# gabrieldemarmiesse/mojo-simdjson

Hardware: AMD Instinct MI355X
Metric: stage-1 GB/s JSON ingested (+ % HBM3E peak), 1/2/4/8 MI355X (higher is better)
Workload: dtype u8

## Files before the change

### mojo_simdjson_amd/csrc/lane_math.h

```cpp
#pragma once
#include <stdint.h>

#if defined(__HIPCC__)
#define MSJ_HD __host__ __device__ __forceinline__
#else
#define MSJ_HD static inline
#endif

namespace msj {

MSJ_HD uint32_t perm(uint32_t s0, uint32_t s1, uint32_t sel) {
#if defined(__HIP_DEVICE_COMPILE__)
    return __builtin_amdgcn_perm(s0, s1, sel);
#else
    uint64_t d = ((uint64_t)s0 << 32) | s1;
    uint32_t r = 0;
    for (int i = 0; i < 4; i++) {
        uint32_t s = (sel >> (8 * i)) & 0xFF;
        r |= (uint32_t)((d >> (8 * (s & 7))) & 0xFF) << (8 * i);
    }
    return r;
#endif
}

// ... 195 lines not shown
#else
    return (uint32_t)__builtin_clzll(inv);
#endif
}

MSJ_HD uint64_t escape_tt0(uint64_t backslash) {
    const uint64_t ODD = 0xAAAAAAAAAAAAAAAAull;
    const uint32_t lo = (uint32_t)backslash, hi = (uint32_t)(backslash >> 32);
    uint32_t sl;
#if defined(__HIP_DEVICE_COMPILE__)
    asm("v_add_u32_e32 %0, %1, %1" : "=v"(sl) : "v"(lo));
    const uint32_t sh = __builtin_amdgcn_alignbit(hi, lo, 31);
#else
    sl = lo << 1;
    const uint32_t sh = (hi << 1) | (lo >> 31);
#endif
    return (u64(sl, sh) | ODD) - backslash;
}
MSJ_HD uint32_t escape_out0(uint64_t tt, uint64_t backslash) {
    return lut3<MSJ_TT((TA ^ TB) & TC)>((uint32_t)(tt >> 32), 0xAAAAAAAAu, (uint32_t)(backslash >> 32)) >> 31;
}
MSJ_HD uint64_t unescaped_quotes0(uint64_t quote_chr, uint64_t tt) {
    return lut3<MSJ_TT(TA & ~(TB ^ TC))>(quote_chr, tt, 0xAAAAAAAAAAAAAAAAull);
}

struct Utf8Leads {
    uint64_t lead234, lead34, lead4;
    uint64_t l3, hi2, f;
};

MSJ_HD Utf8Leads utf8_leads(const uint64_t p[8]) {
    const uint64_t b3 = p[3], b4 = p[4], b5 = p[5], b6 = p[6], b7 = p[7];
    Utf8Leads u;
    u.hi2 = b7 & b6;
    u.f = lut3<MSJ_TT(TA & TB & TC)>(u.hi2, b5, b4);
    u.l3 = lut3<MSJ_TT(TA & TB & ~TC)>(u.hi2, b5, b4);
    u.lead4 = lut3<MSJ_TT(TA & ~TB)>(u.f, b3, b3);
    u.lead234 = lut3<MSJ_TT(TA & ~(TB & TC))>(u.hi2, u.f, b3);
    u.lead34 = u.l3 | u.lead4;
    return u;
}

MSJ_HD uint32_t utf8_special_top(const uint64_t p[8], const Utf8Leads &u) {
    const uint32_t t = 63;
    const uint32_t b0 = (uint32_t)(p[0] >> t) & 1u, b1 = (uint32_t)(p[1] >> t) & 1u, b2 = (uint32_t)(p[2] >> t) & 1u;
    const uint32_t b3 = (uint32_t)(p[3] >> t) & 1u, l3 = (uint32_t)(u.l3 >> t) & 1u, l4 = (uint32_t)(u.lead4 >> t) & 1u;
    const uint32_t z210 = !(b2 | b1 | b0), n101 = b2 & !b1 & b0, n100 = b2 & !b1 & !b0;
    return ((l3 & !b3 & z210) << 6) | ((l3 & b3 & n101) << 7) | ((l4 & z210) << 8) | ((l4 & n100) << 9);
}

MSJ_HD uint32_t utf8_carry_out(const uint64_t p[8], const Utf8Leads &u) {
    return (uint32_t)(u.lead234 >> 63) | ((uint32_t)(u.lead34 >> 62) << 1) | ((uint32_t)(u.lead4 >> 61) << 3) |
           utf8_special_top(p, u);
}

MSJ_HD uint32_t utf8_boundary_error(uint32_t carry_in, uint32_t first_b5, uint32_t first_b4) {
    const uint32_t n5 = first_b5 & 1u, n54 = (first_b5 | first_b4) & 1u;
    return (((carry_in >> 6) & 1u) & (n5 ^ 1u)) |
           (((carry_in >> 7) & 1u) & n5) |
           (((carry_in >> 8) & 1u) & (n54 ^ 1u)) |
           (((carry_in >> 9) & 1u) & n54);
}

template <int K>
MSJ_HD uint64_t shl_in(uint64_t x, uint32_t low) {
    const uint32_t lo = (uint32_t)x, hi = (uint32_t)(x >> 32);
#if defined(__HIP_DEVICE_COMPILE__)
    const uint32_t nh = __builtin_amdgcn_alignbit(hi, lo, 32 - K);
#else
    const uint32_t nh = (hi << K) | (lo >> (32 - K));
#endif
    return u64((lo << K) | low, nh);
}

struct Utf8Shifted {
    uint64_t exp1, exp2, exp3;
    uint64_t nb5, nb54;
};

MSJ_HD uint64_t utf8_errors_shifted(const uint64_t p[8], const Utf8Leads &u, const Utf8Shifted &s, uint64_t *pair_bad) {
    const uint64_t b0 = p[0], b1 = p[1], b2 = p[2], b3 = p[3];
    const uint64_t b4 = p[4], b5 = p[5], b6 = p[6], b7 = p[7];
    const uint64_t cont = lut3<MSJ_TT(TA & ~TB)>(b7, b6, b6);
    const uint64_t e12 = s.exp1 | s.exp2;
    uint64_t err = lut3<MSJ_TT((TA | TB) ^ TC)>(e12, s.exp3, cont);
    const uint64_t x567 = lut3<MSJ_TT(TA & (TB | TC))>(b2, b1, b0);
    const uint64_t f5ff = lut3<MSJ_TT(TA & (TB | TC))>(u.f, b3, x567);
    const uint64_t z432 = lut3<MSJ_TT(~TA & ~TB & ~TC)>(b4, b3, b2);
    const uint64_t w = lut3<MSJ_TT(TA & ~TB & ~TC)>(z432, b1, b5);
    const uint64_t c0c1 = u.hi2 & w;
    err = lut3<MSJ_TT(TA | TB | TC)>(err, f5ff, c0c1);
    const uint64_t z210 = lut3<MSJ_TT(~TA & ~TB & ~TC)>(b2, b1, b0);
    const uint64_t m10 = lut3<MSJ_TT(TA & ~TB)>(b2, b1, b1);
    const uint64_t t1 = lut3<MSJ_TT(TA & ~TB & ~TC)>(u.l3, b3, s.nb5);
    const uint64_t t2 = lut3<MSJ_TT((TA & ~TB) | TC)>(u.lead4, s.nb54, t1);
    const uint64_t u1 = lut3<MSJ_TT(TA & TB & TC)>(u.l3, b3, s.nb5);
    const uint64_t v1 = u.lead4 & s.nb54;
    const uint64_t sel = lut3<MSJ_TT((TC & TA) | (~TC & TB))>(u1, v1, b0);
    const uint64_t lo_bad = z210 & t2;
    *pair_bad = lut3<MSJ_TT(TA | (TB & TC))>(lo_bad, m10, sel);
    return err;
}

MSJ_HD uint64_t utf8_errors(const uint64_t p[8], const Utf8Leads &u, uint32_t carry_in, uint32_t next_b5,
                            uint32_t next_b4, bool have_next) {
    const uint32_t c = carry_in;
// ... 53 lines not shown
```

### mojo_simdjson_amd/csrc/stage1_kernel.hip

```cpp
#include <hip/hip_runtime.h>
#include <stddef.h>
#include <stdint.h>

#include "../../include/msj_stage1.h"
#include "lane_math.h"
#include "stage1_kernel.h"

namespace msj {

constexpr uint32_t kPrioCoord = 2;
constexpr uint32_t kPrioEmit = 3;
constexpr uint32_t kPrioCompute = 0;
constexpr uint32_t kPrioCompute2 = 1;

constexpr uint64_t kAgg = 1ull << 62;
constexpr uint64_t kPre = 2ull << 62;

__device__ __forceinline__ uint64_t ld_desc(const uint64_t *p) {
    return __hip_atomic_load(p, __ATOMIC_RELAXED, __HIP_MEMORY_SCOPE_AGENT);
}
__device__ __forceinline__ void st_desc(uint64_t *p, uint64_t v) {
    __hip_atomic_store(p, v, __ATOMIC_RELAXED, __HIP_MEMORY_SCOPE_AGENT);
}

// ... 92 lines not shown
__device__ __forceinline__ uint32_t cin_internal_error(const KernelArgs &a) {
    return (a.flags & kFlagCarryByValue) ? 0u : a.carry_in->internal_error & 1u;
}
__device__ __forceinline__ msj_carry cin_all(const KernelArgs &a) {
    if (!(a.flags & kFlagCarryByValue)) return *a.carry_in;
    msj_carry c;
    c.count = c.bytes = 0;
    c.in_string = a.carry_bits & 1u;
    c.next_is_escaped = (a.carry_bits >> 1) & 1u;
    c.prev_scalar = (a.carry_bits >> 2) & 1u;
    c.unescaped_error = c.utf8_error = c.internal_error = c.capacity_error = 0;
    c.code = 0;
    for (int k = 0; k < 4; k++) c.reserved[k] = 0;
    return c;
}

struct WaitClock {
    uint32_t spins = 0, t0 = 0;
    __device__ __forceinline__ bool expired(const uint32_t wait_ticks) {
        if ((++spins & 15u) != 0u) return false;
        const uint32_t now = (uint32_t)__builtin_amdgcn_s_memrealtime();
        if (spins == 16u) {
            t0 = now;
            return false;
        }
        return now - t0 > wait_ticks;
    }
    __device__ __forceinline__ void restart() { spins = 0; }
};

__device__ __forceinline__ uint64_t wait_desc(const uint64_t *p, const uint32_t wait_ticks, uint32_t *timeout) {
    uint64_t d = uniform64(ld_desc(p));
    WaitClock clk;
    while ((d >> 62) == 0ull) {
        __builtin_amdgcn_s_sleep(2);
        d = uniform64(ld_desc(p));
        if (clk.expired(wait_ticks)) {
            *timeout = 1;
            break;
        }
    }
    return d;
}

__device__ __forceinline__ void lds_wave_sync_early() {
    asm volatile("s_waitcnt lgkmcnt(0)" ::: "memory");
    __builtin_amdgcn_fence(__ATOMIC_RELEASE, "wavefront");
    __builtin_amdgcn_wave_barrier();
    __builtin_amdgcn_fence(__ATOMIC_ACQUIRE, "wavefront");
}

struct Block {
    uint4 q[4];
    uint32_t wb;
};

template <bool kCoalesced, bool kNt = false>
__device__ __forceinline__ void load_block(const KernelArgs &a, const uint32_t tile, const uint32_t (&lane_off)[4],
                                           const uint32_t lane, Block &b) {
    const uint32_t len32 = (uint32_t)a.len;
    const uint32_t tile_off = tile * kTileBytes;
    const uint8_t *base = a.buf + tile_off;
    const uint32_t lim = ((len32 - 1u) & ~15u) - tile_off;
#pragma unroll
    for (int k = 0; k < 4; k++) {
        const uint32_t off = lane_off[k] < lim ? lane_off[k] : lim;
        if (kCoalesced) {
            typedef uint32_t u32x4 __attribute__((ext_vector_type(4)));
            const u32x4 *src = reinterpret_cast<const u32x4 *>(base + off);
            const u32x4 v = kNt ? __builtin_nontemporal_load(src) : *src;
            b.q[k] = make_uint4(v.x, v.y, v.z, v.w);
        } else {
            b.q[k] = *reinterpret_cast<const uint4 *>(base + off);
        }
    }
    const bool have_window = (tile > 0) || (a.flags & kFlagHasPrefix);
    const uint8_t *wbase = have_window ? base - 64 : a.buf;
    const uint32_t wlim = have_window ? 63u : len32 - 1u;
    b.wb = wbase[lane < wlim ? lane : wlim];
}

struct ChunkAddr {
    uint32_t wr, rd, sw16;
};
__device__ __forceinline__ ChunkAddr chunk_addresses(const uint32_t *stage, const uint32_t lane) {
    const uint32_t s0 = (uint32_t)(uintptr_t)stage;
    ChunkAddr c;
    c.wr = s0 + 64u * (lane >> 2) + 16u * ((lane & 3u) ^ ((lane >> 3) & 3u));
    c.rd = s0 + 64u * lane;
    c.sw16 = 16u * ((lane >> 1) & 3u);
    return c;
}
__device__ __forceinline__ void chunks_to_block(Block &b, const ChunkAddr &ca) {
    typedef uint32_t u32x4 __attribute__((ext_vector_type(4)));
    typedef __attribute__((address_space(3))) u32x4 *lds_u32x4_ptr;
#pragma unroll
    for (int k = 0; k < 4; k++) {
        const u32x4 v = {b.q[k].x, b.q[k].y, b.q[k].z, b.q[k].w};
        *(lds_u32x4_ptr)(uintptr_t)(ca.wr + 1024u * k) = v;
    }
    lds_wave_sync_early();
#pragma unroll
    for (int c = 0; c < 4; c++) {
        const u32x4 v = *(lds_u32x4_ptr)(uintptr_t)(ca.rd + (ca.sw16 ^ (16u * c)));
        b.q[c] = make_uint4(v.x, v.y, v.z, v.w);
    }
}

template <bool kNt>
__device__ __forceinline__ void load_range(const KernelArgs &a, const uint32_t lo, const uint32_t wave,
                                           const uint32_t (&lane_off)[4], const uint32_t lane, Block (&blk)[kBatch]) {
    const uint32_t ntiles = a.ntiles;
#pragma unroll
    for (uint32_t j = 0; j < kBatch; j++) {
        const uint32_t t = lo + kWaves * j + wave;
        load_block<true, kNt>(a, t < ntiles ? t : ntiles - 1u, lane_off, lane, blk[j]);
    }
}
constexpr uint32_t kNtMaxIndices = 3000;
constexpr uint32_t kNtMinTiles = 98304;

__device__ __forceinline__ void touch_block(Block &b) {
#pragma unroll
    for (int k = 0; k < 4; k++)
        asm volatile("" : "+v"(b.q[k].x), "+v"(b.q[k].y), "+v"(b.q[k].z), "+v"(b.q[k].w));
    asm volatile("" : "+v"(b.wb));
}
__device__ __forceinline__ void touch_u64(uint64_t &v) {
    uint32_t lo = (uint32_t)v, hi = (uint32_t)(v >> 32);
    asm volatile("" : "+v"(lo), "+v"(hi));
    v = ((uint64_t)hi << 32) | lo;
}

__device__ __forceinline__ uint32_t ticket_request(unsigned int *ctr, uint32_t lane, uint32_t count) {
    uint32_t ret = 0;
    if (lane == 0)
        asm volatile("global_atomic_add %0, %1, %2, off sc0" : "=v"(ret) : "v"(ctr), "v"(count) : "memory");
    return ret;
}
__device__ __forceinline__ uint32_t ticket_value(uint32_t reg) {
    asm volatile("s_waitcnt vmcnt(0)" ::: "memory");
    return bcast(reg, 0);
}
__device__ __forceinline__ uint32_t ticket_range(uint32_t k, uint32_t shard, uint32_t shards) {
    return (k - (shard == 0u ? 1u : 0u)) * shards + shard;
}

__device__ __forceinline__ void scatter_bits32(uint32_t t, uint32_t lds_byte_addr, uint32_t nbits, uint32_t value_base) {
    uint32_t lo, hi, tm1;
    uint64_t save;
    const uint32_t back = lds_byte_addr + 4u * nbits - 128u;
    const uint32_t vb31 = value_base + 31u;
    const uint32_t topbit = 0x80000000u;
    asm volatile(
        "s_mov_b64 %[save], exec\n"
        ".set msj_sb_k, 0\n"
        ".rept 16\n"
        "v_cmpx_ne_u32_e32 vcc, 0, %[t]\n"
        "s_cbranch_execz 1f\n"
        "v_ffbl_b32_e32 %[lo], %[t]\n"
        "v_ffbh_u32_e32 %[hi], %[t]\n"
        "v_add_u32_e32 %[tm1], -1, %[t]\n"
        "v_or_b32_e32 %[lo], %[lo], %[vb]\n"
        "ds_write_b32 %[front], %[lo] offset:4*msj_sb_k\n"
        "v_sub_u32_e32 %[lo], %[vb31], %[hi]\n"
        "v_lshrrev_b32_e32 %[hi], %[hi], %[top]\n"
        "ds_write_b32 %[back], %[lo] offset:124-4*msj_sb_k\n"
        "v_bitop3_b32 %[t], %[t], %[tm1], %[hi] bitop3:0x40\n"
        ".set msj_sb_k, msj_sb_k+1\n"
        ".endr\n"
        "1:\n"
        "s_mov_b64 exec, %[save]\n"
        : [t] "+v"(t), [lo] "=&v"(lo), [hi] "=&v"(hi), [tm1] "=&v"(tm1), [save] "=&s"(save)
        : [front] "v"(lds_byte_addr), [back] "v"(back), [vb] "v"(value_base), [vb31] "v"(vb31), [top] "v"(topbit)
        : "vcc", "memory");
}

static_assert(offsetof(Shared, stage) >= 128, "scatter_bits32 addresses the back slots from 128 bytes below the lane's end slot");

struct Pending {
    uint64_t T0, T1;
    uint32_t excl;
    uint32_t tile_cnt;
};

struct TileCarry {
    uint32_t e_in, ps_in, u8_in;
    bool resolved;
};
__device__ __forceinline__ TileCarry window_carries(const KernelArgs &a, const uint32_t tile, const uint32_t wb,
                                                    const uint32_t carry0) {
    TileCarry c;
    const bool have_window = (tile > 0) || (a.flags & kFlagHasPrefix);
    const uint32_t b1 = bcast(wb, 63), b2 = bcast(wb, 62), b3 = bcast(wb, 61);
    c.u8_in = 0;
    if (have_window && ((b1 | b2 | b3) & 0x80u)) {
        const uint32_t l1 = (b1 >= 0xC0u && b1 < 0xF8u), l1_34 = (b1 >= 0xE0u && b1 < 0xF8u);
        const uint32_t l1_4 = (b1 >= 0xF0u && b1 < 0xF8u);
        const uint32_t l2_34 = (b2 >= 0xE0u && b2 < 0xF8u), l2_4 = (b2 >= 0xF0u && b2 < 0xF8u);
        const uint32_t l3_4 = (b3 >= 0xF0u && b3 < 0xF8u);
        c.u8_in = l1 | (l2_34 << 1) | (l1_34 << 2) | (l3_4 << 3) | (l2_4 << 4) | (l1_4 << 5) |
                  ((uint32_t)(b1 == 0xE0u) << 6) | ((uint32_t)(b1 == 0xEDu) << 7) |
                  ((uint32_t)(b1 == 0xF0u) << 8) | ((uint32_t)(b1 == 0xF4u) << 9);
    }
    const uint64_t WB = __ballot(wb == 0x5Cu);
    constexpr uint64_t ODD = 0xAAAAAAAAAAAAAAAAull;
    const uint64_t t = (((WB << 1) | ODD) - WB) ^ ODD;
    const uint32_t esc1 = (uint32_t)((t ^ WB) >> 63);
    constexpr uint64_t kNsLo = (1ull << 0x09) | (1ull << 0x0A) | (1ull << 0x0C) | (1ull << 0x0D) |
                               (1ull << 0x1A) | (1ull << 0x20) | (1ull << 0x2C) | (1ull << 0x3A);
    constexpr uint64_t kNsHi = (1ull << (0x5B - 64)) | (1ull << (0x5D - 64)) |
                               (1ull << (0x7B - 64)) | (1ull << (0x7D - 64));
    const uint64_t tab = (b1 & 0x40u) ? kNsHi : kNsLo;
    const uint32_t nonscalar = (uint32_t)(tab >> (b1 & 63u)) & (uint32_t)(b1 < 0x80u);
    c.e_in = (uint32_t)((t & WB) >> 63);
    c.ps_in = ~nonscalar & 1u & ((b1 == 0x22u) ? esc1 : 1u);
    c.resolved = (WB | (1ull << 63)) != ~0ull;
    if (tile == 0) {
        c.e_in = carry0 & 1u;
        c.ps_in = (carry0 >> 1) & 1u;
        c.resolved = true;
    }
    return c;
}

__device__ __forceinline__ Pending compute_tile(const KernelArgs &a, const uint32_t tile,
                                                const uint32_t lane, const Block &blk, const uint32_t carry0,
                                                uint32_t &timeout, uint64_t &agg_word, const uint32_t exact = 0u) {
    const uint32_t len = (uint32_t)a.len;
    MSJ_STAMP(tile, 1);
    uint32_t x[16];
#pragma unroll
    for (int k = 0; k < 4; k++) {
        x[4 * k + 0] = blk.q[k].x;
        x[4 * k + 1] = blk.q[k].y;
        x[4 * k + 2] = blk.q[k].z;
        x[4 * k + 3] = blk.q[k].w;
    }
    TileCarry tc = window_carries(a, tile, blk.wb, carry0);
    if (exact & 1u) {
        tc.e_in = (exact >> 1) & 1u;
        tc.ps_in = (exact >> 2) & 1u;
        tc.resolved = true;
    }
    const uint32_t skip = tile == 0 ? (a.flags >> kFlagSkipShift) & 15u : 0u;
    const bool partial = tile * kTileBytes + kTileBytes > len;

    MSJ_STAMP(tile, 2);
    uint64_t p[8];
    bitplanes(x, p);
    Classes cls;
    uint64_t valid = ~0ull;
    if (!partial && !skip) {
        cls = classify(p, ~0ull);
    } else {
        const uint32_t blk_off = tile * kTileBytes + lane * 64u;
        if (blk_off >= len)
            valid = 0ull;
        else if (len - blk_off < 64u)
            valid = (1ull << (len - blk_off)) - 1ull;
        if (lane == 0) valid &= ~0ull << skip;
#pragma unroll
        for (int k = 0; k < 8; k++) p[k] &= valid;
        cls = classify(p, valid);
    }
    const uint64_t nonascii = __ballot(((uint32_t)p[7] | (uint32_t)(p[7] >> 32)) != 0u);

    const uint64_t qb = cls.quote_chr | cls.backslash;
    const bool quiet = __ballot(((uint32_t)qb | (uint32_t)(qb >> 32)) != 0u) == 0ull && !partial && tc.resolved;
    uint64_t quote = 0, in_string0 = 0, escaped = 0;
    uint32_t tile_e_out = 0, tile_par = 0;
    if (!quiet) {
        const uint64_t tt = escape_tt0(cls.backslash);
        const uint64_t G = __ballot(escape_out0(tt, cls.backslash) != 0u);
        const uint64_t Pm = __ballot(((uint32_t)cls.backslash & (uint32_t)(cls.backslash >> 32)) == 0xFFFFFFFFu);
        quote = unescaped_quotes0(cls.quote_chr, tt);
        const uint64_t add_a = G | Pm, add_b = G;
        uint64_t add_s = add_a + add_b + tc.e_in;
        uint64_t carries = add_s ^ add_a ^ add_b;
        MSJ_STAMP(tile, 3);
        if (carries != 0ull || partial || !tc.resolved) {
            if (!tc.resolved) {
                uint32_t to = 0;
                const uint64_t d = wait_desc(&a.ws[kDescOffset + tile - 1], a.wait_ticks, &to);
                if (to) timeout = 1;
                tc.e_in = (uint32_t)(d >> 58) & 1u;
                tc.ps_in = (uint32_t)(d >> 57) & 1u;
                add_s = add_a + add_b + tc.e_in;
                carries = add_s ^ add_a ^ add_b;
            }
            const uint64_t B0 = __ballot(((uint32_t)cls.backslash & 1u) != 0u);
            if ((carries & B0) == 0ull && !partial) {
                const bool starts_escaped = __builtin_amdgcn_inverse_ballot_w64(carries);
                const uint32_t qlo = (uint32_t)quote;
                quote = u64(starts_escaped ? qlo & ~1u : qlo, (uint32_t)(quote >> 32));
            } else {
                uint32_t lane_e_out;
                escaped = escaped_mask(cls.backslash, (uint32_t)(carries >> lane) & 1u, &lane_e_out);
                quote = cls.quote_chr & ~escaped;
            }
        }
        const uint64_t S0 = prefix_xor(quote);
        tile_e_out = (uint32_t)(((add_a & add_b) | ((add_a | add_b) & ~add_s)) >> 63);
        const uint64_t PM = __ballot((int32_t)(uint32_t)(S0 >> 32) < 0);
        const uint32_t lane_par = lanes_below(PM);
        tile_par = (uint32_t)__popcll(PM) & 1u;
        const uint32_t lane_in32 = (uint32_t)__builtin_amdgcn_sbfe((int)lane_par, 0, 1);
        const uint64_t lane_in = u64(lane_in32, lane_in32);
        in_string0 = S0 ^ lane_in;
    }

    const uint64_t nqs = lut3<MSJ_TT(~TA & ~TB & ~TC)>(cls.op, cls.ws, quote);
    const uint32_t my_ps = (uint32_t)(nqs >> 63);
    const uint32_t prev_ps = dpp_shift_up1(my_ps, tc.ps_in);
    uint32_t tile_ps_out = bcast((uint32_t)(nqs >> 32), 63) >> 31;
    const uint64_t follows = u64(((uint32_t)nqs << 1) | prev_ps, __builtin_amdgcn_alignbit((uint32_t)(nqs >> 32), (uint32_t)nqs, 31));
    const uint64_t potential = lut3<MSJ_TT(TA | (~TB & ~TC))>(cls.op, cls.ws, follows);
    Pending r;
    r.T0 = lut3<MSJ_TT(TA & ~(TB ^ TC))>(potential, in_string0, quote);
    r.T1 = lut3<MSJ_TT(TA & (TB ^ TC))>(potential, in_string0, quote);
    const uint32_t pk = (uint32_t)__popcll(r.T0) | ((uint32_t)__popcll(r.T1) << 16);
    const uint32_t inc = dpp_add_scan(pk);
    r.excl = inc - pk;
    r.tile_cnt = bcast(inc, 63);
    if (partial) {
        const uint32_t lastpos = len - 1u - tile * kTileBytes, ll = lastpos >> 6, lb = lastpos & 63u;
        tile_e_out = bcast((uint32_t)((cls.backslash & ~escaped) >> lb) & 1u, (int)ll);
        tile_ps_out = bcast((uint32_t)(nqs >> lb) & 1u, (int)ll);
    }
    const uint64_t e0 = cls.ctrl & in_string0;
    const uint64_t me0 = __ballot(e0 != 0ull);
    const uint64_t me1 = __ballot(e0 != cls.ctrl);
    MSJ_STAMP(tile, 4);

    uint32_t tile_pend = 0;
// ... 319 lines not shown
            e.mode = kEmitDense;
            return;
        }
        stage_indices_round(e, v, stage, lane64, 0u);
    }
}
template <bool kTypes = false>
__device__ __forceinline__ void emit_store(const KernelArgs &a, const Shared &sh, const EmitU &e, const uint32_t wave,
                                           const uint32_t slot, uint32_t *stage, const uint32_t lane, const uint32_t lane_p) {
    if (e.mode == kEmitStaged) {
        copy_out<kTypes>(a, e, stage, lane, lane_p);
    } else if (e.mode == kEmitStaged2) {
        copy_out<kTypes>(a, emit_round(e, 0u), stage, lane, lane_p);
        lds_wave_sync();
        const EmitV v = emit_lane(sh, wave, slot, lane, e);
        stage_indices_round(e, v, stage, lane64_of(lane), 1u);
        lds_wave_sync();
        copy_out<kTypes>(a, emit_round(e, 1u), stage, lane, lane_p);
    } else if (e.mode == kEmitDense) {
        const EmitV v = emit_lane(sh, wave, slot, lane, e);
        emit_dense<kTypes>(a.idx, e.tile_base, e.base, v.tlo, v.thi, v.vpos - e.shift, lane, a.types, a.buf - a.index_bias);
    } else if (e.mode == kEmitGeneral) {
        const EmitV v = emit_lane(sh, wave, slot, lane, e);
        emit_general<kTypes>(a.idx, a.capacity, e.tile_base, e.base, e.shift, e.vend, v.tlo, v.thi, v.vpos, stage, lane,
                             a.types, a.buf - a.index_bias);
    }
}

template <bool kTypes>
__device__ __forceinline__ void worker_wave(const KernelArgs &a, Shared &sh, const uint32_t lane,
                                            const uint32_t wave) {
    const uint32_t workers = gridDim.x - 1u;
    const uint32_t shards = workers < kTicketShards ? workers : kTicketShards;
    const uint32_t shard = uniform32(sh.shard);
    uint32_t *stage = sh.stage[wave] + kStageSlack;
    const uint32_t tid = threadIdx.x;
    (void)tid;
    const uint32_t lane64 = lane * 64u;
    const uint32_t lane16 = lane * 16u;
    const uint32_t lane_off[4] = {lane16, lane16 + 1024u, lane16 + 2048u, lane16 + 3072u};
    const ChunkAddr chunk_at = chunk_addresses(stage, lane);
    const uint32_t ntiles = a.ntiles;
    const uint32_t nranges = (ntiles + kRange - 1u) / kRange;
    uint64_t *ragg = a.ws + kDescOffset + ntiles;
    const uint64_t *rpre = ragg + nranges;
    if (lane < kPendSlots) sh.pend_meta[wave][lane][0] = 0xFFFFFFFFu;
    MSJ_RSTAMP(a.ntiles + 4096u + blockIdx.x, 2, tid == 0);
    uint32_t lo_cur = uniform32(sh.first_lo);
    const uint64_t count0 = uniform64(cin_count(a));
    const uint32_t carry0 = uniform32(cin_carry0(a));
    uint32_t timeout = 0;

    Block blk[kBatch];
    load_range<false>(a, lo_cur, wave, lane_off, lane, blk);
#pragma unroll
    for (uint32_t j = 0; j < kBatch; j++) touch_block(blk[j]);
    MSJ_RSTAMP(a.ntiles + 4096u + blockIdx.x, 3, tid == 0);

    uint32_t r = 0, ring = 0;
    while (lo_cur < ntiles) {
        uint32_t lane_p = lane, wave_p = wave;
        asm volatile("" : "+v"(lane_p));
        asm volatile("" : "+s"(wave_p));
        KernelArgs al = a;
        asm volatile("" : "+s"(al.flags));
        const uint32_t tid_p = wave_p * 64u + lane_p;
        uint32_t carry0_p = carry0, shard_p = shard;
        asm volatile("" : "+s"(carry0_p), "+s"(shard_p));
        unsigned int *ticket_ctr_p = reinterpret_cast<unsigned int *>(al.ws + (uint64_t)shard_p * kTicketStrideWords);
        const uint32_t par = r & 1u;
        const uint32_t old_first = uniform32(sh.pend_meta[wave][ring * kBatch][0]);
        const bool have_old = old_first != 0xFFFFFFFFu;
        const uint32_t old_range = have_old ? old_first / kRange : 0u;
        uint64_t rp_word = ld_desc(&rpre[old_range]);
        MSJ_RSTAMP(old_range * kRange, 10, tid == 0 && have_old);
        Pending now[kBatch];
        uint32_t req_reg = 0;
#pragma unroll
        for (uint32_t j = 0; j < kBatch; j++) {
            const uint32_t t_cur = lo_cur + kWaves * j + wave;
            const bool valid_tile = t_cur < ntiles;
            MSJ_STAMP(valid_tile ? t_cur : ntiles - 1u, 0);
            uint64_t agg_word = kAgg;
            now[j].T0 = 0;
            now[j].T1 = 0;
            now[j].excl = 0;
            now[j].tile_cnt = 0;
            if (valid_tile) {
                chunks_to_block(blk[j], chunk_at);
                now[j] = compute_tile(al, t_cur, lane, blk[j], carry0_p, timeout, agg_word);
                lds_wave_sync_early();
            }
            if (j == 0) {
                __builtin_amdgcn_s_setprio(kPrioCompute2);
                asm volatile("s_waitcnt vmcnt(0)" ::: "memory");
                touch_u64(rp_word);
                if (tid_p == 0) req_reg = ticket_request(ticket_ctr_p, 0u, 1u);
            }
            if (lane_p == 0) {
                if (valid_tile) st_desc(&a.ws[kDescOffset + t_cur], agg_word);
                sh.tagg[par][kWaves * j + wave] = agg_word;
            }
            MSJ_STAMP(valid_tile ? t_cur : ntiles - 1u, 7);
        }
        const uint32_t srow = (lo_cur + kWaves + wave < ntiles) ? lo_cur + kWaves + wave : ntiles - 1u;
        (void)srow;
        MSJ_STAMP(srow, 8);
        asm volatile("s_waitcnt lgkmcnt(0)\n\ts_barrier" ::: "memory");
        MSJ_STAMP(srow, 9);
        __builtin_amdgcn_s_setprio(kPrioCoord);
        if (wave_p == 0) {
            const uint32_t v = ticket_value(req_reg);
            if (lane_p == 0)
                __hip_atomic_store(&sh.handoff, ((uint64_t)(r + 1u) << 32) | (uint64_t)(ticket_range(v, shard_p, shards) * kRange),
                                   __ATOMIC_RELAXED, __HIP_MEMORY_SCOPE_WORKGROUP);
        }
        uint32_t in_cnt[kBatch], in_state[kBatch];
        {
            const uint64_t w = sh.tagg[par][lane & (kRange - 1u)];
            const uint32_t wl = (uint32_t)w, wh = (uint32_t)(w >> 32);
            const uint32_t P8 = (uint32_t)__ballot((wh & (1u << 29)) != 0u) & 0xFFu;
            const uint32_t s0 = __builtin_amdgcn_mbcnt_lo(P8, 0u) & 1u;
            const uint32_t ab = __builtin_amdgcn_alignbit(wl, wl, s0 << 4);
            uint32_t inc = ab;
            inc += (uint32_t)__builtin_amdgcn_update_dpp(0, (int)inc, 0x111, 0xF, 0xF, false);
            inc += (uint32_t)__builtin_amdgcn_update_dpp(0, (int)inc, 0x112, 0xF, 0xF, false);
            inc += (uint32_t)__builtin_amdgcn_update_dpp(0, (int)inc, 0x114, 0xF, 0xF, false);
            const uint32_t excl = inc - ab;
            const uint32_t anyflag = (uint32_t)__ballot((wh & 0x19400000u) != 0u) & 0xFFu;
            uint32_t e0s = 0, e1s = 0, u8s = 0, pzs = 0;
            if (anyflag) {
                const uint32_t e0 = (wh >> 28) & 1u, e1 = (wh >> 27) & 1u;
                e0s = ((uint32_t)__ballot((s0 ? e1 : e0) != 0u) & 0xFFu) != 0u;
                e1s = ((uint32_t)__ballot((s0 ? e0 : e1) != 0u) & 0xFFu) != 0u;
                u8s = ((uint32_t)__ballot(((wh >> 24) & 1u) != 0u) & 0xFFu) != 0u;
                pzs = ((uint32_t)__ballot(((wh >> 22) & 1u) != 0u) & 0xFFu) != 0u;
            }
#pragma unroll
            for (uint32_t j = 0; j < kBatch; j++) {
                const uint32_t k = kWaves * j + wave;
                in_cnt[j] = bcast(excl, (int)k);
                const uint32_t sk = (uint32_t)__builtin_popcount(P8 & ((1u << k) - 1u)) & 1u;
                in_state[j] = sk | ((sk ^ 1u) << 1);
            }
            if (tid_p == 0) {
                const uint32_t tot = bcast(inc, (int)kRange - 1);
                const uint32_t s_out = (uint32_t)__builtin_popcount(P8) & 1u;
                st_desc(&ragg[lo_cur / kRange], kAgg | ((uint64_t)s_out << 61) | ((uint64_t)e0s << 60) |
                                                    ((uint64_t)e1s << 59) | ((uint64_t)u8s << 56) |
                                                    ((uint64_t)pzs << 54) | ((uint64_t)(tot >> 16) << 16) |
                                                    (uint64_t)(tot & 0xFFFFu));
            }
        }
        if (al.ws_clean && wave_p == kWaves - 1) {
            const uint32_t rid = lo_cur / kRange;
            if (lane_p < kRange) {
                if (lo_cur + lane < ntiles) al.ws_clean[kDescOffset + lo_cur + lane] = 0ull;
            } else if (lane_p == kRange) {
                al.ws_clean[kDescOffset + ntiles + rid] = 0ull;
            } else if (lane_p == kRange + 1u) {
                al.ws_clean[kDescOffset + ntiles + nranges + rid] = 0ull;
            }
        }
        MSJ_STAMP(srow, 10);
        uint32_t lo_next;
        {
            uint64_t h = uniform64(__hip_atomic_load(&sh.handoff, __ATOMIC_RELAXED, __HIP_MEMORY_SCOPE_WORKGROUP));
            WaitClock clk;
            while ((uint32_t)(h >> 32) != r + 1u) {
                __builtin_amdgcn_s_sleep(1);
                h = uniform64(__hip_atomic_load(&sh.handoff, __ATOMIC_RELAXED, __HIP_MEMORY_SCOPE_WORKGROUP));
                if (clk.expired(al.wait_ticks)) {
                    timeout = 1;
                    h = ((uint64_t)(r + 1u) << 32) | 0xFFFFFFFFull;
                }
            }
            lo_next = (uint32_t)h;
        }
        {
            const uint32_t c0 = now[0].tile_cnt, c1 = now[1].tile_cnt;
            const uint32_t n0 = (c0 & 0xFFFFu) > (c0 >> 16) ? (c0 & 0xFFFFu) : (c0 >> 16);
            const uint32_t n1 = (c1 & 0xFFFFu) > (c1 >> 16) ? (c1 & 0xFFFFu) : (c1 >> 16);
            if (uniform32(n0 + n1) > kNtMaxIndices || ntiles < kNtMinTiles) {
                load_range<false>(a, lo_next, wave, lane_off, lane, blk);
            } else {
                asm volatile("; non-temporal range loads");
                load_range<true>(a, lo_next, wave, lane_off, lane, blk);
                asm volatile("; end of non-temporal range loads");
            }
        }
        MSJ_RSTAMP(lo_cur, 8, tid == 0);
        if (have_old) {
            rp_word = range_prefix(al, rpre, old_range, uniform64(rp_word), timeout);
            MSJ_RSTAMP(old_range * kRange, 9, tid == 0);
        }
        const uint64_t rp = uniform64(rp_word);
        timeout = uniform32(timeout);
        MSJ_STAMP(srow, 12);
        static_assert(kBatch == 2, "the emission below is written for two tiles per wave and range");
        __builtin_amdgcn_s_setprio(kPrioEmit);
        const uint32_t slot0 = ring * kBatch;
        EmitU e0 = emit_prepare(al, sh, wave, slot0, rp, count0, timeout);
        emit_stage(sh, e0, wave, slot0, stage, lane, lane64);
        lds_wave_sync();
        MSJ_STAMP(srow, 13);
        emit_store<kTypes>(al, sh, e0, wave, slot0, stage, lane, lane_p);
        lds_wave_sync();
        MSJ_STAMP(srow, 14);
        EmitU e1 = emit_prepare(al, sh, wave, slot0 + 1u, rp, count0, timeout);
        emit_stage(sh, e1, wave, slot0 + 1u, stage, lane, lane64);
        lds_wave_sync();
        MSJ_STAMP(srow, 15);
        asm volatile("s_waitcnt vmcnt(0)" ::: "memory");
#pragma unroll
        for (uint32_t j = 0; j < kBatch; j++) touch_block(blk[j]);
        MSJ_STAMP(srow, 11);
        emit_store<kTypes>(al, sh, e1, wave, slot0 + 1u, stage, lane, lane_p);
        lds_wave_sync();
        __builtin_amdgcn_s_setprio(kPrioCompute);
#pragma unroll
        for (uint32_t j = 0; j < kBatch; j++) {
            const uint32_t slot = slot0 + j;
            const uint32_t t_cur = lo_cur + kWaves * j + wave;
            sh.pend_masks[wave][slot][lane] = make_uint4((uint32_t)now[j].T0, (uint32_t)(now[j].T0 >> 32),
                                                         (uint32_t)now[j].T1, (uint32_t)(now[j].T1 >> 32));
            sh.pend_excl[wave][slot][lane] = now[j].excl;
            if (lane_p == 0)
                *reinterpret_cast<uint4 *>(sh.pend_meta[wave][slot]) =
                    make_uint4(t_cur < ntiles ? t_cur : 0xFFFFFFFFu, now[j].tile_cnt, in_cnt[j], in_state[j]);
        }
        lo_cur = lo_next;
        r++;
        ring = (ring + 1u == kDefer) ? 0u : ring + 1u;
    }
    MSJ_RSTAMP(a.ntiles + 4096u + blockIdx.x, 4, tid == 0);
    __builtin_amdgcn_s_setprio(kPrioEmit);
    for (uint32_t step = 0; step < kDefer; step++) {
        lds_wave_sync();
        const uint32_t old_first = uniform32(sh.pend_meta[wave][ring * kBatch][0]);
        if (old_first != 0xFFFFFFFFu) {
            const uint64_t w = uniform64(range_prefix(a, rpre, old_first / kRange, 0ull, timeout));
            timeout = uniform32(timeout);
#pragma unroll
            for (uint32_t j = 0; j < kBatch; j++) {
                const uint32_t slot = ring * kBatch + j;
                EmitU e = emit_prepare(a, sh, wave, slot, w, count0, timeout);
                emit_stage(sh, e, wave, slot, stage, lane, lane64);
                lds_wave_sync();
                emit_store<kTypes>(a, sh, e, wave, slot, stage, lane, lane);
                lds_wave_sync();
            }
        }
        ring = (ring + 1u == kDefer) ? 0u : ring + 1u;
    }
    MSJ_RSTAMP(a.ntiles + 4096u + blockIdx.x, 5, tid == 0);
    if (uniform32(timeout) && lane == 0) atomicOr(&a.carry_out->internal_error, 1u);
}

__device__ __forceinline__ void finish_launch(const KernelArgs &a, const uint32_t cs, const uint32_t cc,
                                              const uint32_t ce, const uint32_t cu, const uint32_t cx,
                                              const uint64_t *tile_agg = nullptr, const bool late_poison = false) {
    const msj_carry cin = cin_all(a);
    if (!tile_agg) tile_agg = a.ws + kDescOffset;
    const uint64_t last = ld_desc(&tile_agg[a.ntiles - 1u]);
    const bool do_utf8 = !(a.flags & kFlagNoUtf8);
    msj_carry out;
    const uint64_t n = cin.count + cc;
    out.count = n;
    out.bytes = cin.bytes + a.len;
    out.in_string = cs;
    out.next_is_escaped = (uint32_t)(last >> 58) & 1u;
    out.prev_scalar = (uint32_t)(last >> 57) & 1u;
    out.unescaped_error = (cin.unescaped_error | ce) ? 1u : 0u;
    uint32_t u8e = cin.utf8_error | cu;
    if ((a.flags & kFlagFinal) && do_utf8 && (a.len % kTileBytes) == 0 && ((last >> 55) & 1u)) u8e = 1;
    out.utf8_error = u8e ? 1u : 0u;
// ... 201 lines not shown
#pragma unroll
                for (int e = 0; e < kResolveE; e++) {
                    const uint32_t lo_e = (uint32_t)e * 64u;
                    if (lo_e < m) {
                        const uint32_t nact = (m - lo_e) < 64u ? (m - lo_e) : 64u;
                        const bool act = lane < nact;
                        const uint64_t de = act ? d[e] : kAgg;
                        const uint32_t p = (uint32_t)(de >> 61) & 1u;
                        const uint32_t c0 = (uint32_t)de & 0xFFFFu, c1 = (uint32_t)(de >> 16) & 0xFFFFu;
                        const uint32_t e0 = (uint32_t)(de >> 60) & 1u, e1 = (uint32_t)(de >> 59) & 1u;
                        const uint64_t PM = __ballot(p != 0u);
                        const uint32_t in_l = cs ^ ((uint32_t)__popcll(PM & below) & 1u);
                        const uint32_t mine = in_l ? c1 : c0;
                        const uint32_t incl = dpp_add_scan(mine);
                        const uint64_t EM = __ballot((in_l ? e1 : e0) != 0u);
                        const uint64_t U = __ballot(((de >> 56) & 1ull) != 0ull);
                        const uint64_t X = __ballot(((de >> 54) & 1ull) != 0ull);
                        const uint32_t t = base + lo_e + lane;
                        if (act && lo_e + lane >= published && t < ntiles) {
                            const uint32_t e_in = ce | (((EM & below) != 0ull) ? 1u : 0u);
                            const uint32_t u_in = cu | (((U & below) != 0ull) ? 1u : 0u);
                            const uint64_t pz = (uint64_t)((cx | (((X & below) != 0ull) ? 1u : 0u) |
                                                            ((uint32_t)(de >> 54) & 1u))) << 54;
                            st_desc(&pre[t], kPre | ((uint64_t)in_l << 61) | ((uint64_t)e_in << 60) |
                                                 ((uint64_t)u_in << 56) | pz | (uint64_t)(cc + incl - mine));
                            }
                        cc += bcast(incl, 63);
                        ce |= EM ? 1u : 0u;
                        cu |= U ? 1u : 0u;
                        cs ^= (uint32_t)__popcll(PM) & 1u;
                    }
                }
                published = m;
                clk.restart();
            }
            if (clk.expired(a.wait_ticks)) force = 1;
            if (!full) __builtin_amdgcn_s_sleep(1);
        }
    }
}


constexpr uint64_t kTpUnresolved = 3ull << 62;

__global__ __launch_bounds__(kThreads) void twopass_summary_kernel(const KernelArgs a) {
    const uint32_t lane = threadIdx.x & 63u, wave = uniform32(threadIdx.x >> 6);
    const uint32_t tile = blockIdx.x * kWaves + wave;
    if (tile >= a.ntiles) return;
    const uint32_t lane64 = lane * 64u;
    const uint32_t lane_off[4] = {lane64, lane64 + 16u, lane64 + 32u, lane64 + 48u};
    const uint32_t carry0 = uniform32(cin_carry0(a));
    Block blk;
    load_block<false>(a, tile, lane_off, lane, blk);
    uint64_t *tp = a.tp;
    if (!window_carries(a, tile, blk.wb, carry0).resolved) {
        if (lane == 0) tp[tile] = kTpUnresolved;
        return;
    }
    uint32_t timeout = 0;
    uint64_t agg_word;
    (void)compute_tile(a, tile, lane, blk, carry0, timeout, agg_word);
    if (lane == 0) tp[tile] = agg_word;
}

__global__ __launch_bounds__(64) void twopass_scan_kernel(const KernelArgs a) {
    const uint32_t lane = threadIdx.x;
    const uint32_t ntiles = a.ntiles;
    uint64_t *agg = a.tp, *pre = a.tp + ntiles;
    const uint32_t lane64 = lane * 64u;
    const uint32_t lane_off[4] = {lane64, lane64 + 16u, lane64 + 32u, lane64 + 48u};
    const uint32_t carry0 = uniform32(cin_carry0(a));
    const uint64_t below = (1ull << lane) - 1ull;
    uint32_t cs = uniform32(cin_in_string(a)), cc = 0, ce = 0, cu = 0;
    uint32_t e_prev = carry0 & 1u, ps_prev = (carry0 >> 1) & 1u;
    for (uint32_t base = 0; base < ntiles; base += 64u) {
        const uint32_t t = base + lane;
        uint64_t w = t < ntiles ? agg[t] : kAgg;
        const uint64_t unres = __ballot((w >> 62) == 3ull);
        if (unres == 0ull) {
            const uint32_t p = (uint32_t)(w >> 61) & 1u;
            const uint32_t c0 = (uint32_t)w & 0xFFFFu, c1 = (uint32_t)(w >> 16) & 0xFFFFu;
            const uint32_t e0 = (uint32_t)(w >> 60) & 1u, e1 = (uint32_t)(w >> 59) & 1u;
            const uint64_t PM = __ballot(p != 0u);
            const uint32_t in_l = cs ^ ((uint32_t)__popcll(PM & below) & 1u);
            const uint32_t mine = in_l ? c1 : c0;
            const uint32_t incl = dpp_add_scan(mine);
            const uint64_t EM = __ballot((in_l ? e1 : e0) != 0u);
            const uint64_t U = __ballot(((w >> 56) & 1ull) != 0ull);
            if (t < ntiles) pre[t] = kPre | ((uint64_t)in_l << 61) | (uint64_t)(cc + incl - mine);
            cc += bcast(incl, 63);
            ce |= EM ? 1u : 0u;
            cu |= U ? 1u : 0u;
            cs ^= (uint32_t)__popcll(PM) & 1u;
            const uint32_t last = (ntiles - base < 64u ? ntiles - base : 64u) - 1u;
            const uint32_t wh = bcast((uint32_t)(w >> 32), (int)last);
            e_prev = (wh >> 26) & 1u;
            ps_prev = (wh >> 25) & 1u;
        } else {
            const uint32_t cnt = ntiles - base < 64u ? ntiles - base : 64u;
            for (uint32_t k = 0; k < cnt; k++) {
                uint64_t wk = u64(bcast((uint32_t)w, (int)k), bcast((uint32_t)(w >> 32), (int)k));
                uint32_t exact = 0;
                if ((wk >> 62) == 3ull) {
                    Block blk;
                    load_block<false>(a, base + k, lane_off, lane, blk);
                    uint32_t timeout = 0;
                    exact = 1u | (e_prev << 1) | (ps_prev << 2);
                    (void)compute_tile(a, base + k, lane, blk, carry0, timeout, wk, exact);
                    if (lane == 0) agg[base + k] = wk;
                }
                const uint32_t c = cs ? (uint32_t)(wk >> 16) & 0xFFFFu : (uint32_t)wk & 0xFFFFu;
                if (lane == 0) pre[base + k] = kPre | ((uint64_t)cs << 61) | ((uint64_t)exact << 50) | (uint64_t)cc;
                cc += c;
                ce |= (uint32_t)(wk >> (cs ? 59 : 60)) & 1u;
                cu |= (uint32_t)(wk >> 56) & 1u;
                cs ^= (uint32_t)(wk >> 61) & 1u;
                e_prev = (uint32_t)(wk >> 58) & 1u;
                ps_prev = (uint32_t)(wk >> 57) & 1u;
            }
        }
    }
    __builtin_amdgcn_fence(__ATOMIC_RELEASE, "agent");
    if (lane == 0) finish_launch(a, cs, cc, ce, cu, 0u, agg);
}

__global__ __launch_bounds__(kThreads) void twopass_emit_kernel(const KernelArgs a) {
    __shared__ Shared sh;
    const uint32_t lane = threadIdx.x & 63u, wave = uniform32(threadIdx.x >> 6);
    const uint32_t tile = blockIdx.x * kWaves + wave;
    if (tile >= a.ntiles) return;
    const uint32_t lane64 = lane * 64u;
    const uint32_t lane_off[4] = {lane64, lane64 + 16u, lane64 + 32u, lane64 + 48u};
    const uint32_t carry0 = uniform32(cin_carry0(a));
    const uint64_t count0 = uniform64(cin_count(a));
    Block blk;
    load_block<false>(a, tile, lane_off, lane, blk);
    const uint64_t pw = uniform64(a.tp[a.ntiles + tile]);
    uint32_t timeout = 0;
    uint64_t agg_word;
    const Pending r = compute_tile(a, tile, lane, blk, carry0, timeout, agg_word, (uint32_t)(pw >> 50) & 7u);
    const uint32_t s_in = (uint32_t)(pw >> 61) & 1u;
    sh.pend_masks[wave][0][lane] = make_uint4((uint32_t)r.T0, (uint32_t)(r.T0 >> 32), (uint32_t)r.T1, (uint32_t)(r.T1 >> 32));
    sh.pend_excl[wave][0][lane] = r.excl;
    if (lane == 0) *reinterpret_cast<uint4 *>(sh.pend_meta[wave][0]) = make_uint4(tile, r.tile_cnt, 0u, s_in | (s_in << 1));
    lds_wave_sync();
    uint32_t *stage = sh.stage[wave] + kStageSlack;
    EmitU e = emit_prepare(a, sh, wave, 0, kPre | (uint64_t)(uint32_t)pw, count0, timeout);
    emit_stage(sh, e, wave, 0, stage, lane, lane64);
    lds_wave_sync();
    emit_store(a, sh, e, wave, 0, stage, lane, lane);
}

template <bool kTypes>
__device__ __forceinline__ void stage1_body(const KernelArgs &a) {
    __shared__ Shared sh;
    const uint32_t tid = threadIdx.x;
    MSJ_RSTAMP(a.ntiles + 4096u + blockIdx.x, 0, tid == 0);
    if (tid == 0) {
        const uint32_t workers = gridDim.x - 1u;
        const uint32_t shards = workers < kTicketShards ? workers : kTicketShards;
        const uint32_t shard = (gridDim.x >= 8u * kTicketShards ? blockIdx.x >> 3 : blockIdx.x) % shards;
        const uint32_t k = atomicAdd(reinterpret_cast<unsigned int *>(a.ws + (uint64_t)shard * kTicketStrideWords), 1u);
        sh.role = (shard == 0u && k == 0u) ? 0u : 1u;
        sh.shard = shard;
        sh.first_lo = ticket_range(k, shard, shards) * kRange;
        sh.handoff = 0ull;
    }
    __syncthreads();
    if (sh.role == 0u) {
        resolver(a, sh);
        return;
    }
    worker_wave<kTypes>(a, sh, tid & 63u, uniform32(tid >> 6));
}
__global__ __launch_bounds__(kThreads, 4) void stage1_kernel(const KernelArgs a) { stage1_body<false>(a); }
__global__ __launch_bounds__(kThreads, 4) void stage1_types_kernel(const KernelArgs a) { stage1_body<true>(a); }

}

extern "C" int msj_launch_stage1(const msj::KernelArgs *args, void *stream, uint32_t grid) {
    const msj::KernelArgs a = *args;
    const uint32_t need = (a.ntiles + msj::kWaves - 1u) / msj::kWaves + 1u;
    const uint32_t g = (grid == 0 || grid > need) ? need : grid;
    if (a.flags & msj::kFlagEmitTypes)
        hipLaunchKernelGGL(msj::stage1_types_kernel, dim3(g < 2u ? 2u : g), dim3(msj::kThreads), 0, static_cast<hipStream_t>(stream), a);
    else
        hipLaunchKernelGGL(msj::stage1_kernel, dim3(g < 2u ? 2u : g), dim3(msj::kThreads), 0, static_cast<hipStream_t>(stream), a);
    return (int)hipGetLastError();
}

extern "C" int msj_launch_stage1_twopass(const msj::KernelArgs *args, void *stream) {
    const msj::KernelArgs a = *args;
    hipStream_t s = static_cast<hipStream_t>(stream);
// ... 12 lines not shown
```

Before: 3434.

## Assign contiguous tile pairs per wave and hand carries from first tile to second

Tile assignment within a range changes from strided (wave + kWaves*j) to contiguous (kBatch*wave + j), so each wave processes adjacent tiles. The second tile's escape/scalar/UTF-8 carries are computed directly from the first tile's aggregate word and last bytes, instead of loading a 64-byte window and possibly spin-waiting on the previous tile's descriptor. Only one window load per batch is issued, and only the last tile of each wave publishes its descriptor. This serialises the two tiles' carry dependency within a wave. It also changes the order in which descriptors appear for cross-wave lookback, which could lengthen waits for the next wave's first tile.

```diff
diff --git a/mojo_simdjson_amd/csrc/lane_math.h b/mojo_simdjson_amd/csrc/lane_math.h
--- a/mojo_simdjson_amd/csrc/lane_math.h
+++ b/mojo_simdjson_amd/csrc/lane_math.h
@@ -271,6 +271,26 @@
 MSJ_HD uint32_t utf8_carry_out(const uint64_t p[8], const Utf8Leads &u) {
     return (uint32_t)(u.lead234 >> 63) | ((uint32_t)(u.lead34 >> 62) << 1) | ((uint32_t)(u.lead4 >> 61) << 3) |
            utf8_special_top(p, u);
+}
+
+MSJ_HD uint32_t utf8_carry_of_bytes(uint32_t b1, uint32_t b2, uint32_t b3) {
+    const uint32_t l1 = (b1 >= 0xC0u && b1 < 0xF8u), l1_34 = (b1 >= 0xE0u && b1 < 0xF8u);
+    const uint32_t l1_4 = (b1 >= 0xF0u && b1 < 0xF8u);
+    const uint32_t l2_34 = (b2 >= 0xE0u && b2 < 0xF8u), l2_4 = (b2 >= 0xF0u && b2 < 0xF8u);
+    const uint32_t l3_4 = (b3 >= 0xF0u && b3 < 0xF8u);
+    return l1 | (l2_34 << 1) | (l1_34 << 2) | (l3_4 << 3) | (l2_4 << 4) | (l1_4 << 5) |
+           ((uint32_t)(b1 == 0xE0u) << 6) | ((uint32_t)(b1 == 0xEDu) << 7) |
+           ((uint32_t)(b1 == 0xF0u) << 8) | ((uint32_t)(b1 == 0xF4u) << 9);
+}
+
+MSJ_HD uint32_t prev_scalar_of_byte(uint32_t b1, uint32_t escaped) {
+    constexpr uint64_t kNsLo = (1ull << 0x09) | (1ull << 0x0A) | (1ull << 0x0C) | (1ull << 0x0D) |
+                               (1ull << 0x1A) | (1ull << 0x20) | (1ull << 0x2C) | (1ull << 0x3A);
+    constexpr uint64_t kNsHi = (1ull << (0x5B - 64)) | (1ull << (0x5D - 64)) |
+                               (1ull << (0x7B - 64)) | (1ull << (0x7D - 64));
+    const uint64_t tab = (b1 & 0x40u) ? kNsHi : kNsLo;
+    const uint32_t nonscalar = (uint32_t)(tab >> (b1 & 63u)) & (uint32_t)(b1 < 0x80u);
+    return ~nonscalar & 1u & ((b1 == 0x22u) ? escaped : 1u);
 }
 
 MSJ_HD uint32_t utf8_boundary_error(uint32_t carry_in, uint32_t first_b5, uint32_t first_b4) {
diff --git a/mojo_simdjson_amd/csrc/stage1_kernel.hip b/mojo_simdjson_amd/csrc/stage1_kernel.hip
--- a/mojo_simdjson_amd/csrc/stage1_kernel.hip
+++ b/mojo_simdjson_amd/csrc/stage1_kernel.hip
@@ -168,7 +168,6 @@
 
 struct Block {
     uint4 q[4];
-    uint32_t wb;
 };
 
 template <bool kCoalesced, bool kNt = false>
@@ -190,10 +189,14 @@
             b.q[k] = *reinterpret_cast<const uint4 *>(base + off);
         }
     }
+}
+__device__ __forceinline__ uint32_t load_window(const KernelArgs &a, const uint32_t tile, const uint32_t lane) {
+    const uint32_t len32 = (uint32_t)a.len;
+    const uint8_t *base = a.buf + tile * kTileBytes;
     const bool have_window = (tile > 0) || (a.flags & kFlagHasPrefix);
     const uint8_t *wbase = have_window ? base - 64 : a.buf;
     const uint32_t wlim = have_window ? 63u : len32 - 1u;
-    b.wb = wbase[lane < wlim ? lane : wlim];
+    return wbase[lane < wlim ? lane : wlim];
 }
 
 struct ChunkAddr {
@@ -225,12 +228,15 @@
 
 template <bool kNt>
 __device__ __forceinline__ void load_range(const KernelArgs &a, const uint32_t lo, const uint32_t wave,
-                                           const uint32_t (&lane_off)[4], const uint32_t lane, Block (&blk)[kBatch]) {
+                                           const uint32_t (&lane_off)[4], const uint32_t lane, Block (&blk)[kBatch],
+                                           uint32_t &wb) {
     const uint32_t ntiles = a.ntiles;
 #pragma unroll
     for (uint32_t j = 0; j < kBatch; j++) {
-        const uint32_t t = lo + kWaves * j + wave;
-        load_block<true, kNt>(a, t < ntiles ? t : ntiles - 1u, lane_off, lane, blk[j]);
+        const uint32_t t = lo + kBatch * wave + j;
+        const uint32_t tc = t < ntiles ? t : ntiles - 1u;
+        load_block<true, kNt>(a, tc, lane_off, lane, blk[j]);
+        if (j == 0) wb = load_window(a, tc, lane);
     }
 }
 constexpr uint32_t kNtMaxIndices = 3000;
@@ -240,8 +246,8 @@
 #pragma unroll
     for (int k = 0; k < 4; k++)
         asm volatile("" : "+v"(b.q[k].x), "+v"(b.q[k].y), "+v"(b.q[k].z), "+v"(b.q[k].w));
-    asm volatile("" : "+v"(b.wb));
-}
+}
+__device__ __forceinline__ void touch_u32(uint32_t &v) { asm volatile("" : "+v"(v)); }
 __device__ __forceinline__ void touch_u64(uint64_t &v) {
     uint32_t lo = (uint32_t)v, hi = (uint32_t)(v >> 32);
     asm volatile("" : "+v"(lo), "+v"(hi));
@@ -310,27 +316,13 @@
     const bool have_window = (tile > 0) || (a.flags & kFlagHasPrefix);
     const uint32_t b1 = bcast(wb, 63), b2 = bcast(wb, 62), b3 = bcast(wb, 61);
     c.u8_in = 0;
-    if (have_window && ((b1 | b2 | b3) & 0x80u)) {
-        const uint32_t l1 = (b1 >= 0xC0u && b1 < 0xF8u), l1_34 = (b1 >= 0xE0u && b1 < 0xF8u);
-        const uint32_t l1_4 = (b1 >= 0xF0u && b1 < 0xF8u);
-        const uint32_t l2_34 = (b2 >= 0xE0u && b2 < 0xF8u), l2_4 = (b2 >= 0xF0u && b2 < 0xF8u);
-        const uint32_t l3_4 = (b3 >= 0xF0u && b3 < 0xF8u);
-        c.u8_in = l1 | (l2_34 << 1) | (l1_34 << 2) | (l3_4 << 3) | (l2_4 << 4) | (l1_4 << 5) |
-                  ((uint32_t)(b1 == 0xE0u) << 6) | ((uint32_t)(b1 == 0xEDu) << 7) |
-                  ((uint32_t)(b1 == 0xF0u) << 8) | ((uint32_t)(b1 == 0xF4u) << 9);
-    }
+    if (have_window && ((b1 | b2 | b3) & 0x80u)) c.u8_in = utf8_carry_of_bytes(b1, b2, b3);
     const uint64_t WB = __ballot(wb == 0x5Cu);
     constexpr uint64_t ODD = 0xAAAAAAAAAAAAAAAAull;
     const uint64_t t = (((WB << 1) | ODD) - WB) ^ ODD;
     const uint32_t esc1 = (uint32_t)((t ^ WB) >> 63);
-    constexpr uint64_t kNsLo = (1ull << 0x09) | (1ull << 0x0A) | (1ull << 0x0C) | (1ull << 0x0D) |
-                               (1ull << 0x1A) | (1ull << 0x20) | (1ull << 0x2C) | (1ull << 0x3A);
-    constexpr uint64_t kNsHi = (1ull << (0x5B - 64)) | (1ull << (0x5D - 64)) |
-                               (1ull << (0x7B - 64)) | (1ull << (0x7D - 64));
-    const uint64_t tab = (b1 & 0x40u) ? kNsHi : kNsLo;
-    const uint32_t nonscalar = (uint32_t)(tab >> (b1 & 63u)) & (uint32_t)(b1 < 0x80u);
     c.e_in = (uint32_t)((t & WB) >> 63);
-    c.ps_in = ~nonscalar & 1u & ((b1 == 0x22u) ? esc1 : 1u);
+    c.ps_in = prev_scalar_of_byte(b1, esc1);
     c.resolved = (WB | (1ull << 63)) != ~0ull;
     if (tile == 0) {
         c.e_in = carry0 & 1u;
@@ -340,9 +332,22 @@
     return c;
 }
 
+__device__ __forceinline__ TileCarry pair_handover(const uint64_t first_agg, const uint32_t first_tail) {
+    TileCarry c;
+    c.e_in = (uint32_t)(first_agg >> 58) & 1u;
+    c.ps_in = (uint32_t)(first_agg >> 57) & 1u;
+    c.u8_in = 0;
+    if (first_tail & 0x80808000u) c.u8_in = utf8_carry_of_bytes(first_tail >> 24, (first_tail >> 16) & 0xFFu, (first_tail >> 8) & 0xFFu);
+    c.resolved = true;
+    return c;
+}
+
+template <bool kHanded = false>
 __device__ __forceinline__ Pending compute_tile(const KernelArgs &a, const uint32_t tile,
-                                                const uint32_t lane, const Block &blk, const uint32_t carry0,
-                                                uint32_t &timeout, uint64_t &agg_word, const uint32_t exact = 0u) {
+                                                const uint32_t lane, const Block &blk, const uint32_t wb,
+                                                const uint32_t carry0, uint32_t &timeout, uint64_t &agg_word,
+                                                const uint32_t exact = 0u, const TileCarry *handed = nullptr,
+                                                uint32_t *tail = nullptr) {
     const uint32_t len = (uint32_t)a.len;
     MSJ_STAMP(tile, 1);
     uint32_t x[16];
@@ -353,8 +358,14 @@
         x[4 * k + 2] = blk.q[k].z;
         x[4 * k + 3] = blk.q[k].w;
     }
-    TileCarry tc = window_carries(a, tile, blk.wb, carry0);
-    if (exact & 1u) {
+    TileCarry tc;
+    if (kHanded) {
+        tc = *handed;
+        tc.resolved = true;
+    } else {
+        tc = window_carries(a, tile, wb, carry0);
+    }
+    if (!kHanded && (exact & 1u)) {
         tc.e_in = (exact >> 1) & 1u;
         tc.ps_in = (exact >> 2) & 1u;
         tc.resolved = true;
@@ -381,6 +392,7 @@
         cls = classify(p, valid);
     }
     const uint64_t nonascii = __ballot(((uint32_t)p[7] | (uint32_t)(p[7] >> 32)) != 0u);
+    if (tail) *tail = nonascii != 0ull ? bcast(x[15], 63) : 0u;
 
     const uint64_t qb = cls.quote_chr | cls.backslash;
     const bool quiet = __ballot(((uint32_t)qb | (uint32_t)(qb >> 32)) != 0u) == 0ull && !partial && tc.resolved;
@@ -395,8 +407,8 @@
         uint64_t add_s = add_a + add_b + tc.e_in;
         uint64_t carries = add_s ^ add_a ^ add_b;
         MSJ_STAMP(tile, 3);
-        if (carries != 0ull || partial || !tc.resolved) {
-            if (!tc.resolved) {
+        if (carries != 0ull || partial || (!kHanded && !tc.resolved)) {
+            if (!kHanded && !tc.resolved) {
                 uint32_t to = 0;
                 const uint64_t d = wait_desc(&a.ws[kDescOffset + tile - 1], a.wait_ticks, &to);
                 if (to) timeout = 1;
@@ -822,9 +834,11 @@
     uint32_t timeout = 0;
 
     Block blk[kBatch];
-    load_range<false>(a, lo_cur, wave, lane_off, lane, blk);
+    uint32_t wb;
+    load_range<false>(a, lo_cur, wave, lane_off, lane, blk, wb);
 #pragma unroll
     for (uint32_t j = 0; j < kBatch; j++) touch_block(blk[j]);
+    touch_u32(wb);
     MSJ_RSTAMP(a.ntiles + 4096u + blockIdx.x, 3, tid == 0);
 
     uint32_t r = 0, ring = 0;
@@ -846,9 +860,10 @@
         MSJ_RSTAMP(old_range * kRange, 10, tid == 0 && have_old);
         Pending now[kBatch];
         uint32_t req_reg = 0;
+        TileCarry hand;
 #pragma unroll
         for (uint32_t j = 0; j < kBatch; j++) {
-            const uint32_t t_cur = lo_cur + kWaves * j + wave;
+            const uint32_t t_cur = lo_cur + kBatch * wave + j;
             const bool valid_tile = t_cur < ntiles;
             MSJ_STAMP(valid_tile ? t_cur : ntiles - 1u, 0);
             uint64_t agg_word = kAgg;
@@ -858,7 +873,13 @@
             now[j].tile_cnt = 0;
             if (valid_tile) {
                 chunks_to_block(blk[j], chunk_at);
-                now[j] = compute_tile(al, t_cur, lane, blk[j], carry0_p, timeout, agg_word);
+                if (j == 0) {
+                    uint32_t tail;
+                    now[j] = compute_tile(al, t_cur, lane, blk[j], wb, carry0_p, timeout, agg_word, 0u, nullptr, &tail);
+                    hand = pair_handover(agg_word, tail);
+                } else {
+                    now[j] = compute_tile<true>(al, t_cur, lane, blk[j], 0u, carry0_p, timeout, agg_word, 0u, &hand);
+                }
                 lds_wave_sync_early();
             }
             if (j == 0) {
@@ -868,12 +889,12 @@
                 if (tid_p == 0) req_reg = ticket_request(ticket_ctr_p, 0u, 1u);
             }
             if (lane_p == 0) {
-                if (valid_tile) st_desc(&a.ws[kDescOffset + t_cur], agg_word);
-                sh.tagg[par][kWaves * j + wave] = agg_word;
+                if (valid_tile && (j == kBatch - 1u || t_cur == ntiles - 1u)) st_desc(&a.ws[kDescOffset + t_cur], agg_word);
+                sh.tagg[par][kBatch * wave + j] = agg_word;
             }
             MSJ_STAMP(valid_tile ? t_cur : ntiles - 1u, 7);
         }
-        const uint32_t srow = (lo_cur + kWaves + wave < ntiles) ? lo_cur + kWaves + wave : ntiles - 1u;
+        const uint32_t srow = (lo_cur + kBatch * wave + 1u < ntiles) ? lo_cur + kBatch * wave + 1u : ntiles - 1u;
         (void)srow;
         MSJ_STAMP(srow, 8);
         asm volatile("s_waitcnt lgkmcnt(0)\n\ts_barrier" ::: "memory");
@@ -908,7 +929,7 @@
             }
 #pragma unroll
             for (uint32_t j = 0; j < kBatch; j++) {
-                const uint32_t k = kWaves * j + wave;
+                const uint32_t k = kBatch * wave + j;
                 in_cnt[j] = bcast(excl, (int)k);
                 const uint32_t sk = (uint32_t)__builtin_popcount(P8 & ((1u << k) - 1u)) & 1u;
                 in_state[j] = sk | ((sk ^ 1u) << 1);
@@ -952,10 +973,10 @@
             const uint32_t n0 = (c0 & 0xFFFFu) > (c0 >> 16) ? (c0 & 0xFFFFu) : (c0 >> 16);
             const uint32_t n1 = (c1 & 0xFFFFu) > (c1 >> 16) ? (c1 & 0xFFFFu) : (c1 >> 16);
             if (uniform32(n0 + n1) > kNtMaxIndices || ntiles < kNtMinTiles) {
-                load_range<false>(a, lo_next, wave, lane_off, lane, blk);
+                load_range<false>(a, lo_next, wave, lane_off, lane, blk, wb);
             } else {
                 asm volatile("; non-temporal range loads");
-                load_range<true>(a, lo_next, wave, lane_off, lane, blk);
+                load_range<true>(a, lo_next, wave, lane_off, lane, blk, wb);
                 asm volatile("; end of non-temporal range loads");
             }
         }
@@ -984,6 +1005,7 @@
         asm volatile("s_waitcnt vmcnt(0)" ::: "memory");
 #pragma unroll
         for (uint32_t j = 0; j < kBatch; j++) touch_block(blk[j]);
+        touch_u32(wb);
         MSJ_STAMP(srow, 11);
         emit_store<kTypes>(al, sh, e1, wave, slot0 + 1u, stage, lane, lane_p);
         lds_wave_sync();
@@ -991,7 +1013,7 @@
 #pragma unroll
         for (uint32_t j = 0; j < kBatch; j++) {
             const uint32_t slot = slot0 + j;
-            const uint32_t t_cur = lo_cur + kWaves * j + wave;
+            const uint32_t t_cur = lo_cur + kBatch * wave + j;
             sh.pend_masks[wave][slot][lane] = make_uint4((uint32_t)now[j].T0, (uint32_t)(now[j].T0 >> 32),
                                                          (uint32_t)now[j].T1, (uint32_t)(now[j].T1 >> 32));
             sh.pend_excl[wave][slot][lane] = now[j].excl;
@@ -1299,14 +1321,15 @@
     const uint32_t carry0 = uniform32(cin_carry0(a));
     Block blk;
     load_block<false>(a, tile, lane_off, lane, blk);
+    const uint32_t wb = load_window(a, tile, lane);
     uint64_t *tp = a.tp;
-    if (!window_carries(a, tile, blk.wb, carry0).resolved) {
+    if (!window_carries(a, tile, wb, carry0).resolved) {
         if (lane == 0) tp[tile] = kTpUnresolved;
         return;
     }
     uint32_t timeout = 0;
     uint64_t agg_word;
-    (void)compute_tile(a, tile, lane, blk, carry0, timeout, agg_word);
+    (void)compute_tile(a, tile, lane, blk, wb, carry0, timeout, agg_word);
     if (lane == 0) tp[tile] = agg_word;
 }
 
@@ -1351,9 +1374,10 @@
                 if ((wk >> 62) == 3ull) {
                     Block blk;
                     load_block<false>(a, base + k, lane_off, lane, blk);
+                    const uint32_t wb = load_window(a, base + k, lane);
                     uint32_t timeout = 0;
                     exact = 1u | (e_prev << 1) | (ps_prev << 2);
-                    (void)compute_tile(a, base + k, lane, blk, carry0, timeout, wk, exact);
+                    (void)compute_tile(a, base + k, lane, blk, wb, carry0, timeout, wk, exact);
                     if (lane == 0) agg[base + k] = wk;
                 }
                 const uint32_t c = cs ? (uint32_t)(wk >> 16) & 0xFFFFu : (uint32_t)wk & 0xFFFFu;
@@ -1382,10 +1406,11 @@
     const uint64_t count0 = uniform64(cin_count(a));
     Block blk;
     load_block<false>(a, tile, lane_off, lane, blk);
+    const uint32_t wb = load_window(a, tile, lane);
     const uint64_t pw = uniform64(a.tp[a.ntiles + tile]);
     uint32_t timeout = 0;
     uint64_t agg_word;
-    const Pending r = compute_tile(a, tile, lane, blk, carry0, timeout, agg_word, (uint32_t)(pw >> 50) & 7u);
+    const Pending r = compute_tile(a, tile, lane, blk, wb, carry0, timeout, agg_word, (uint32_t)(pw >> 50) & 7u);
     const uint32_t s_in = (uint32_t)(pw >> 61) & 1u;
     sh.pend_masks[wave][0][lane] = make_uint4((uint32_t)r.T0, (uint32_t)(r.T0 >> 32), (uint32_t)r.T1, (uint32_t)(r.T1 >> 32));
     sh.pend_excl[wave][0][lane] = r.excl;
```

After: 3437, median of 3. Within noise of the previous version (+0.1%).
